# qdrant/qdrant

Hardware: NVIDIA H100
Metric: queries/sec, 10Mx768 f32 brute-force cosine top-10, single query (GB/s scanned = value * 30.72) (higher is better)
Workload: dtype f32 results (exact reference arithmetic); the scan itself runs on an int8 shadow plane and re-scores the survivors in f32

## Files before the change

qdrant_b200/csrc/qb_localk.cuh:

```cuda
#pragma once
#include "qb_common.cuh"

namespace {

constexpr int QB_LOCALK_SLOTS = 16;
constexpr int QB_LOCALK_WARPS = 8;

__device__ __forceinline__ unsigned long long warp_min_u64(unsigned long long v) {
#pragma unroll
    for (int o = 16; o > 0; o >>= 1) {
        const unsigned long long w = __shfl_xor_sync(0xFFFFFFFFu, v, o);
        v = w < v ? w : v;
    }
    return v;
}

struct LkState { unsigned long long my_key, wmin; float wthr; };
__device__ __noinline__ void lk_push(const uint32_t* deleted, const uint32_t* deleted2, uint32_t id_base, float sc, uint32_t id, unsigned long long* queue,
                                     unsigned int* count) {
    bool dead = false;
    if (deleted) dead = (deleted[id >> 5] >> (id & 31)) & 1u;
    if (deleted2) dead = dead || ((deleted2[id >> 5] >> (id & 31)) & 1u);
    if (!dead) queue[atomicAdd(count, 1u)] = qb_pack_key(sc, id + id_base);
}
__device__ __noinline__ LkState lk_drain(LkState st, const unsigned long long* queue, unsigned int* count, int lane, unsigned int n_queued) {
    for (unsigned int j = 0; j < n_queued; ++j) {
        const unsigned long long k_new = queue[j];
        if (k_new > st.wmin) {
            const unsigned int holders = __ballot_sync(0xFFFFFFFFu, st.my_key == st.wmin);
            if (lane == __ffs((int)holders) - 1) st.my_key = k_new;
            st.wmin = warp_min_u64(st.my_key);
        }
    }
    __syncwarp();
    if (lane == 0) *count = 0u;
    __syncwarp();
    st.wthr = (st.wmin != 0ull) ? qb_key_score(st.wmin) : __int_as_float(0xff800000);
    return st;
}

__device__ __forceinline__ void lk_cta_sort(unsigned long long* lists, int lane) {
    constexpr int N = QB_LOCALK_WARPS * QB_LOCALK_SLOTS;
    for (int k = 2; k <= N; k <<= 1)
        for (int j = k >> 1; j > 0; j >>= 1) {
            for (int i = lane; i < N; i += 32) {
                const int ixj = i ^ j;
                if (ixj > i) {
                    const unsigned long long a = lists[i], b = lists[ixj];
                    const bool desc = ((i & k) == 0);
                    if (desc ? (a < b) : (a > b)) { lists[i] = b; lists[ixj] = a; }
                }
            }
            __syncwarp();
        }
}

__device__ __forceinline__ void lk_last_cta_merge(const unsigned long long* all, uint32_t local_k, qb_scored_point* final_out, uint32_t* final_count,
                                                  unsigned int* done_counter, int lane) {
    __threadfence();
    __syncwarp();
    unsigned int ticket = 0;
    if (lane == 0) ticket = atomicAdd(done_counter, 1u);
    ticket = __shfl_sync(0xFFFFFFFFu, ticket, 0);
    if (ticket != gridDim.x - 1) return;
    __threadfence();
    constexpr int PER = 8;
    unsigned int pos[PER];
    unsigned long long head[PER];
#pragma unroll
    for (int i = 0; i < PER; ++i) {
        const unsigned int l = lane + 32u * i;
        pos[i] = 0;
        head[i] = (l < gridDim.x) ? __ldcg(all + (unsigned long long)l * QB_LOCALK_SLOTS) : 0ull;
    }
    unsigned int n_out = 0;
    for (unsigned int r = 0; r < local_k; ++r) {
        unsigned long long best = 0ull;
        int bi = 0;
#pragma unroll
        for (int i = 0; i < PER; ++i) if (head[i] > best) { best = head[i]; bi = i; }
        unsigned long long wbest = best;
#pragma unroll
        for (int o = 16; o > 0; o >>= 1) { const unsigned long long w = __shfl_xor_sync(0xFFFFFFFFu, wbest, o); wbest = w > wbest ? w : wbest; }
        if (wbest == 0ull) break;
        if (best == wbest) {
#pragma unroll
            for (int i = 0; i < PER; ++i)
                if (i == bi) {
                    pos[i] += 1;
                    const unsigned int l = lane + 32u * i;
                    head[i] = (pos[i] < (unsigned int)QB_LOCALK_SLOTS) ? __ldcg(all + (unsigned long long)l * QB_LOCALK_SLOTS + pos[i]) : 0ull;
                }
            qb_scored_point sp;
            sp.idx = qb_key_id(wbest); sp.score = qb_key_score(wbest);
            final_out[r] = sp;
        }
        n_out = r + 1;
    }
    if (lane == 0) { *final_count = n_out; *done_counter = 0u; }
}

}
```

qdrant_b200/csrc/qb_prefilter.cu:

```cuda
#include <algorithm>

#include "qb_internal.h"
#include "qb_localk.cuh"
#include "qb_score.cuh"

qb_status qb_dense_f32_scan_localk(const qb_storage* s, const QbScanArgs& a, uint32_t top, uint64_t* n_slots, cudaStream_t stream, uint64_t min_rows = 65536);

namespace {

constexpr int PF_CONSUMER_WARPS = 8;
constexpr int PF_MAX_PRODUCERS = 4;
constexpr int PF_PRODUCERS = 2;
constexpr int PF_THREADS = 32 * (PF_CONSUMER_WARPS + PF_MAX_PRODUCERS);
constexpr uint32_t PF_SLOT_BYTES = 12288;
constexpr uint32_t PF_CAP = 131072;
constexpr uint32_t PF_LIST_CAP = 1u << 21;

static int pf_producers() { const int o = qb_opt().prefilter_producers; return (o >= 1 && o <= PF_MAX_PRODUCERS) ? o : PF_PRODUCERS; }

struct PfParams {
    const uint8_t* rows;
    uint32_t stride;
    uint32_t row_h;
    uint32_t dim;
// ... 355 lines not shown
            if (valid) {
                *reinterpret_cast<uint16_t*>(dst + d_pad / 2 + 2 * v) = (uint16_t)hi;
                *reinterpret_cast<uint16_t*>(lo + 2 * v) = (uint16_t)lw;
            }
        }
        if (valid && t == 0) {
            float* meta = reinterpret_cast<float*>(dst + d_pad / 2 + d_pad / 8);
            meta[0] = sr;
            meta[1] = __double2float_ru(__dmul_ru(sqrt(rr5), 1.0 + 0x1p-40));
            meta[2] = __double2float_ru(__dmul_ru(sqrt(rr6), 1.0 + 0x1p-40));
            for (uint32_t b = d_pad / 2 + d_pad / 8 + 12; b < out_stride_b; ++b) dst[b] = 0;
            for (uint32_t b = d_pad / 8; b < lo_b; ++b) lo[b] = 0;
            if (bad || !(ss <= 3.0e38)) atomicOr(nonfinite, 1u);
            else atomicMax(max_norm_bits, __float_as_uint(__double2float_ru(__dmul_ru(sqrt(ss), 1.0 + 0x1p-40))));
        }
    }
}

struct Pf6Params {
    const uint8_t* rows;
    const uint8_t* lo;
    uint32_t stride;
    uint32_t d_pad;
    uint32_t dim;
    uint64_t n_rows;
    const float* q;
    uint32_t rows_per_slot, n_slots, slot_bytes;
    qb_scored_point* samp_out; uint32_t* samp_cnt; uint32_t top;
    const unsigned int* max_norm_bits;
    float* up5;
    uint64_t sample_rows;
    const uint8_t* f32_rows; uint32_t f32_stride; uint32_t id_base;
    unsigned long long* cta_keys; unsigned int* samp_ticket;
    uint32_t* list; unsigned int* list_cnt; unsigned int* list_ticket; uint32_t list_cap;
    uint32_t* cand; unsigned int* cnt; uint32_t cap;
    const uint32_t* deleted; const uint32_t* deleted2;
    int l2_keep;
};

template <int NCH>
struct Q6Query {
    uint32_t hq[NCH][4], lq[NCH][4];
    int sum_h, sum_l;
    float sq, e1, e1_5, t2a, t2b, thr_adj;
};

template <int NCH>
__device__ __forceinline__ void q6_query(const Pf6Params& p, int hl, Q6Query<NCH>& Q) {
    const uint32_t n16 = p.d_pad / 16;
    float qmax = 0.f, q1 = 0.f, q2 = 0.f;
    bool qbad = false;
#pragma unroll
    for (int c = 0; c < NCH; ++c) {
        const uint32_t v = (uint32_t)(c * 16 + hl);
#pragma unroll
        for (int k = 0; k < 16; ++k) {
            const float x = (v < n16 && v * 16 + k < p.dim) ? p.q[v * 16 + k] : 0.f;
            qbad |= !(fabsf(x) <= 3.0e38f);
            qmax = fmaxf(qmax, fabsf(x)); q1 = __fadd_ru(q1, fabsf(x)); q2 = __fmaf_rn(x, x, q2);
        }
    }
#pragma unroll
    for (int o = 8; o; o >>= 1) {
        qmax = fmaxf(qmax, __shfl_xor_sync(0xFFFFFFFFu, qmax, o)); q1 = __fadd_ru(q1, __shfl_xor_sync(0xFFFFFFFFu, q1, o)); q2 += __shfl_xor_sync(0xFFFFFFFFu, q2, o);
        qbad |= __shfl_xor_sync(0xFFFFFFFFu, (int)qbad, o) != 0;
    }
    qbad |= (qmax > 0.f && qmax < 1.0e-30f);
    const float sq = (qmax > 0.f) ? __fdiv_rn(qmax, 127.f) : 0.f;
// ... 286 lines not shown
        s += PF_CONSUMER_WARPS;
        if (s >= p.n_slots) { s -= p.n_slots; ph ^= 1u; }
    }
    if (lane < QB_LOCALK_SLOTS) lists[cw * QB_LOCALK_SLOTS + lane] = (lk.my_key == ~0ull) ? 0ull : lk.my_key;
    asm volatile("bar.sync 1, %0;" ::"n"(PF_CONSUMER_WARPS * 32) : "memory");
    if (cw == 0) lk_cta_sort(lists, lane);
    asm volatile("bar.sync 1, %0;" ::"n"(PF_CONSUMER_WARPS * 32) : "memory");
    if (cw < QB_LOCALK_SLOTS / 4) {
        const int i = cw * 4 + (lane >> 3);
        const unsigned long long k = (i < (int)p.top) ? lists[i] : 0ull;
        const uint32_t row = k ? qb_key_id(k) : 0u;
        const float sc = qbs::score_avx_group8<qbs::M_DOT>(reinterpret_cast<const float*>(p.f32_rows + (size_t)row * p.f32_stride), p.q, p.dim, lane & 7);
        if ((lane & 7) == 0) ex[i] = k ? qb_pack_key(sc, row + p.id_base) : 0ull;
    }
    asm volatile("bar.sync 1, %0;" ::"n"(PF_CONSUMER_WARPS * 32) : "memory");
    if (cw == 0) {
        if (lane < QB_LOCALK_SLOTS) {
            const unsigned long long k = ex[lane];
            int rank = 0;
#pragma unroll
            for (int j = 0; j < QB_LOCALK_SLOTS; ++j) rank += (ex[j] > k || (ex[j] == k && j < lane)) ? 1 : 0;
            p.cta_keys[(unsigned long long)blockIdx.x * QB_LOCALK_SLOTS + rank] = k;
        }
        lk_last_cta_merge(p.cta_keys, p.top, p.samp_out, p.samp_cnt, p.samp_ticket, lane);
    }
}

template <int NCH>
__global__ void __launch_bounds__(PF_THREADS, 1) dense_q5_filter_kernel(const Pf6Params p) { stage1_run<NCH, Q6Query<NCH>>(p); }

template <int NCH>
__global__ void __launch_bounds__(PF_THREADS, 1) dense_q4b_filter_kernel(const Pf6Params p) { stage1_run<NCH, Q4bQuery<NCH>>(p); }

constexpr int PF_COMPACT_THREADS = 256;
template <int NCH>
__global__ void __launch_bounds__(PF_COMPACT_THREADS) dense_q5_compact_kernel(const Pf6Params p) {
    constexpr int UNROLL = 4;
    constexpr int WARPS = PF_COMPACT_THREADS / 32;
    __shared__ float s_thr;
    __shared__ unsigned int s_warp[WARPS], s_base;
    if (threadIdx.x < 32) {
        Q6Query<NCH> Q;
        q6_query<NCH>(p, threadIdx.x & 15, Q);
        if (threadIdx.x == 0) s_thr = Q.thr_adj;
    }
    __syncthreads();
    const float thr_adj = s_thr;
    const int lane = threadIdx.x & 31, warp = threadIdx.x >> 5;
    const uint64_t n4 = (p.n_rows + 3) / 4, step = (uint64_t)gridDim.x * PF_COMPACT_THREADS * UNROLL;
    for (uint64_t b = (uint64_t)blockIdx.x * PF_COMPACT_THREADS * UNROLL; b < n4; b += step) {
        float4 u4[UNROLL];
#pragma unroll
        for (int j = 0; j < UNROLL; ++j) {
            const uint64_t i = b + (uint64_t)j * PF_COMPACT_THREADS + threadIdx.x;
            u4[j] = (i < n4) ? __ldcs(reinterpret_cast<const float4*>(p.up5) + i) : make_float4(0.f, 0.f, 0.f, 0.f);
        }
        uint32_t mask = 0;
#pragma unroll
        for (int j = 0; j < UNROLL; ++j) {
            const uint64_t i = b + (uint64_t)j * PF_COMPACT_THREADS + threadIdx.x;
            const float u[4] = {u4[j].x, u4[j].y, u4[j].z, u4[j].w};
#pragma unroll
            for (int k = 0; k < 4; ++k) {
                const uint64_t row = 4 * i + k;
                if (row < p.n_rows && !(u[k] < thr_adj)) {
                    const uint32_t id = (uint32_t)row;
                    bool dead = false;
                    if (p.deleted) dead = (p.deleted[id >> 5] >> (id & 31)) & 1u;
                    if (p.deleted2) dead = dead || ((p.deleted2[id >> 5] >> (id & 31)) & 1u);
                    mask |= dead ? 0u : 1u << (4 * j + k);
                }
            }
        }
        const int c = __popc(mask);
        int incl = c;
#pragma unroll
        for (int o = 1; o < 32; o <<= 1) { const int t = __shfl_up_sync(0xFFFFFFFFu, incl, o); if (lane >= o) incl += t; }
        if (lane == 31) s_warp[warp] = (unsigned int)incl;
        __syncthreads();
        if (threadIdx.x == 0) {
            unsigned int total = 0;
#pragma unroll
            for (int w = 0; w < WARPS; ++w) { const unsigned int t = s_warp[w]; s_warp[w] = total; total += t; }
            s_base = total ? atomicAdd(p.list_cnt, total) : 0u;
        }
        __syncthreads();
        if (mask) {
            unsigned int pos = s_base + s_warp[warp] + (unsigned int)(incl - c);
            for (uint32_t m = mask; m; m &= m - 1) {
                const int bit = __ffs((int)m) - 1;
                if (pos < p.list_cap) p.list[pos] = (uint32_t)(4 * (b + (uint64_t)(bit >> 2) * PF_COMPACT_THREADS + threadIdx.x) + (bit & 3));
                ++pos;
            }
        }
        __syncthreads();
    }
}

constexpr int PF_RESCREEN_THREADS = 256;
template <int NCH>
__global__ void __launch_bounds__(PF_RESCREEN_THREADS) dense_q6_rescreen_kernel(const Pf6Params p) {
    __shared__ uint4 s_hq[NCH * 16], s_lq[NCH * 16];
    __shared__ float s_k[5];
    __shared__ int s_corr[2];
    __shared__ unsigned int s_n;
    if (threadIdx.x == 0) {
        s_n = *reinterpret_cast<volatile unsigned int*>(p.list_cnt);
        __threadfence();
        if (atomicAdd(p.list_ticket, 1u) == gridDim.x - 1) { *p.list_cnt = 0u; *p.list_ticket = 0u; }
    }
    if (threadIdx.x < 32) {
        const int hl = threadIdx.x & 15;
        Q6Query<NCH> Q;
        q6_query<NCH>(p, hl, Q);
        if (threadIdx.x < 16) {
#pragma unroll
            for (int c = 0; c < NCH; ++c) {
                s_hq[c * 16 + hl] = make_uint4(Q.hq[c][0], Q.hq[c][1], Q.hq[c][2], Q.hq[c][3]);
                s_lq[c * 16 + hl] = make_uint4(Q.lq[c][0], Q.lq[c][1], Q.lq[c][2], Q.lq[c][3]);
            }
        }
        if (threadIdx.x == 0) {
            s_k[0] = Q.sq; s_k[1] = Q.e1; s_k[2] = Q.t2a; s_k[3] = Q.t2b; s_k[4] = Q.thr_adj;
            s_corr[0] = 31 * Q.sum_h; s_corr[1] = 31 * Q.sum_l;
        }
    }
    __syncthreads();
    const unsigned int n1 = s_n;
    if (n1 > p.list_cap) {
        if (blockIdx.x == 0 && threadIdx.x == 0) *p.cnt = p.cap + 1u;
        return;
    }
    const float sq = s_k[0], e1 = s_k[1], t2a = s_k[2], t2b = s_k[3], thr_adj = s_k[4];
    const int corr_h = s_corr[0], corr_l = s_corr[1];
    const float k254 = 1.0f / 254.0f;
    const int lane = threadIdx.x & 31, half = lane >> 4, hl = lane & 15;
    uint32_t hq[NCH][4], lq[NCH][4];
#pragma unroll
    for (int c = 0; c < NCH; ++c) {
        const uint4 h = s_hq[c * 16 + hl], l = s_lq[c * 16 + hl];
        hq[c][0] = h.x; hq[c][1] = h.y; hq[c][2] = h.z; hq[c][3] = h.w;
        lq[c][0] = l.x; lq[c][1] = l.y; lq[c][2] = l.z; lq[c][3] = l.w;
    }
    const uint32_t n16 = p.d_pad / 16, lo_b = q6_lo_stride(p.d_pad);
    const uint32_t a_off = (uint32_t)hl * 8, b_off = p.d_pad / 2 + (uint32_t)hl * 2, meta_off = p.d_pad / 2 + p.d_pad / 8;
    const uint32_t warps = gridDim.x * (blockDim.x >> 5), gw = blockIdx.x * (blockDim.x >> 5) + (threadIdx.x >> 5);
    for (uint32_t e0 = 2 * gw; e0 < n1; e0 += 2 * warps) {
        const uint32_t e = e0 + (uint32_t)half;
        const bool valid = e < n1;
        const uint32_t row = __ldcg(p.list + (valid ? e : e0));
        const uint8_t* rec = p.rows + (size_t)row * p.stride;
        const uint8_t* lo = p.lo + (size_t)row * lo_b;
        int hs = 0, ls = 0;
#pragma unroll
        for (int c = 0; c < NCH; ++c) {
            if ((uint32_t)(c * 16 + hl) < n16) {
                const uint2 x = __ldg(reinterpret_cast<const uint2*>(rec + a_off + 128 * c));
                const uint32_t y = q6_spread(__ldg(reinterpret_cast<const unsigned short*>(rec + b_off + 32 * c)));
                const uint32_t z = q6_spread(__ldg(reinterpret_cast<const unsigned short*>(lo + 2 * hl + 32 * c)));
                const uint32_t w[4] = {((x.x << 1) & 0x1E1E1E1Eu) | (y & 0x01010101u),        ((x.x >> 3) & 0x1E1E1E1Eu) | ((y >> 1) & 0x01010101u),
                                       ((x.y << 1) & 0x1E1E1E1Eu) | ((y >> 2) & 0x01010101u), ((x.y >> 3) & 0x1E1E1E1Eu) | ((y >> 3) & 0x01010101u)};
#pragma unroll
                for (int m = 0; m < 4; ++m) {
                    const uint32_t u = (w[m] << 1) | ((z >> m) & 0x01010101u);
                    hs = __dp4a((int)u, (int)hq[c][m], hs); ls = __dp4a((int)u, (int)lq[c][m], ls);
                }
            }
        }
        int v = ((hl & 8) ? ls : hs) + __shfl_xor_sync(0xFFFFFFFFu, (hl & 8) ? hs : ls, 8);
        v += __shfl_xor_sync(0xFFFFFFFFu, v, 4);
        v += __shfl_xor_sync(0xFFFFFFFFu, v, 2);
        v += __shfl_xor_sync(0xFFFFFFFFu, v, 1);
        const int lsum = __shfl_xor_sync(0xFFFFFFFFu, v, 8);
        if (hl == 0 && valid) {
            const float* meta = reinterpret_cast<const float*>(rec + meta_off);
            const float H = (float)(v - corr_h), L = (float)(lsum - corr_l);
            const float sr = __ldg(meta), rho6 = __ldg(meta + 2);
            const float app = __fmul_rn(sr, __fmul_rn(sq, __fmaf_rn(L, k254, H)));
            const float up = __fadd_ru(app, fminf(__fmul_ru(sr, e1), __fmaf_ru(rho6, t2a, t2b)));
            if (!(up < thr_adj)) {
                const unsigned int pos = atomicAdd(p.cnt, 1u);
                if (pos < p.cap) p.cand[pos] = row;
            }
        }
    }
}

template <typename P>
qb_status launch_ring(void (*kernel)(P), P& p, int sm_count, cudaStream_t stream, size_t extra_smem = 0, uint32_t row_step = 2) {
    const uint32_t kMaxSmem = 227 * 1024;
    const uint32_t target = qb_opt().prefilter_slot_bytes ? qb_opt().prefilter_slot_bytes : PF_SLOT_BYTES;
    uint32_t rps = target / p.stride / row_step * row_step;
    if (rps < row_step) rps = row_step;
    p.rows_per_slot = rps;
    p.slot_bytes = rps * p.stride;
    uint32_t n_slots = (kMaxSmem - 2048 - (uint32_t)extra_smem) / p.slot_bytes;
    if (n_slots > 64) n_slots = 64;
    n_slots = (n_slots / PF_CONSUMER_WARPS) * PF_CONSUMER_WARPS;
    QB_CHECK(n_slots >= (uint32_t)PF_CONSUMER_WARPS, QB_ERR_INVALID, "prefilter: rows too wide for the ring");
    p.n_slots = n_slots;
    const size_t smem = (size_t)n_slots * p.slot_bytes + (size_t)n_slots * 16 + extra_smem;
    QB_CUDA(cudaFuncSetAttribute(kernel, cudaFuncAttributeMaxDynamicSharedMemorySize, (int)kMaxSmem));
    const uint64_t n_tiles = ceil_div_u64(p.n_rows, p.rows_per_slot);
    const unsigned grid = (unsigned)std::min<uint64_t>(n_tiles, (uint64_t)sm_count);
    kernel<<<grid, 32 * (PF_CONSUMER_WARPS + pf_producers()), smem, stream>>>(p);
    QB_LAUNCHED();
    QB_CUDA(cudaGetLastError());
    return QB_OK;
}

template <bool GLOBAL>
__device__ unsigned long long block_next_key(const unsigned long long* k, uint32_t n, unsigned long long prev, unsigned long long* s_best) {
    const int warp = threadIdx.x >> 5, lane = threadIdx.x & 31;
    unsigned long long best = 0ull;
    for (uint32_t i = threadIdx.x; i < n; i += blockDim.x) {
        const unsigned long long x = GLOBAL ? __ldcg(k + i) : k[i];
        if (x < prev && x > best) best = x;
    }
#pragma unroll
    for (int o = 16; o; o >>= 1) { const unsigned long long w = __shfl_xor_sync(0xFFFFFFFFu, best, o); best = w > best ? w : best; }
// ... 116 lines not shown
    }
    s->q4b_row_b = row_b;
    const uint64_t blocks = std::min<uint64_t>(ceil_div_u64(std::max<uint64_t>(s->count, 1), 32), (uint64_t)s->sm_count * 16);
    f32_to_q4b_rows_kernel<<<(unsigned)blocks, 256, 0, stream>>>(reinterpret_cast<const float*>(s->d_rows), s->row_stride / 4, s->dim, d_pad, s->count, s->d_q4b, row_b);
    QB_LAUNCHED();
    QB_CUDA(cudaGetLastError());
    QB_CUDA(cudaStreamSynchronize(stream));
    s->q4b_ready = true;
    return QB_OK;
}

static bool pf_stage1_q4b() { return qb_opt().prefilter_stage1 != 5; }

static int pf_plane() { const int o = qb_opt().prefilter_plane; return (o == 1 || o == 2) ? o : 0; }

bool qb_f32_prefilter_usable(qb_storage* s, uint64_t n_rows, uint32_t top, cudaStream_t stream) {
    if (s->kind != QB_KIND_DENSE || s->dtype != QB_DT_F32) return false;
    if (s->distance != QB_DIST_DOT && s->distance != QB_DIST_COSINE) return false;
    if (qb_opt().disable_prefilter || n_rows != s->count || n_rows < (1ull << 19) || top > 16 || s->dim < 32 || round_up_u64(s->dim, 8) > 1024) return false;
    if (pf_plane() == 0) {
        if (q6_shadow_ensure(s, stream) == QB_OK) {
            if (s->q6_usable && pf_stage1_q4b() && q4b_shadow_ensure(s, stream) != QB_OK) cudaGetLastError();
            return s->q6_usable;
        }
        cudaGetLastError();
    } else if (pf_plane() == 2) {
        if (q8_shadow_ensure(s, stream) == QB_OK) return s->q8_usable;
        cudaGetLastError();
    }
    if (qb_f32_shadow_ensure(s, stream) != QB_OK) { cudaGetLastError(); return false; }
    return s->bf16_usable;
}

size_t qb_f32_prefilter_scratch_bytes() { return 256 + (size_t)PF_CAP * 12 + (size_t)PF_LIST_CAP * 4; }

qb_status qb_f32_prefilter_search(qb_storage* s, const QbScanArgs& a, uint32_t top, void* d_scratch, float* d_up5, unsigned int* d_n_fallbacks, qb_scored_point* d_out,
                                  uint32_t* d_out_cnt, cudaEvent_t prof0, cudaEvent_t prof1, cudaStream_t stream) {
    uint8_t* sc = reinterpret_cast<uint8_t*>(d_scratch);
    unsigned int* d_cnt = reinterpret_cast<unsigned int*>(sc);
    unsigned int* d_fallback = reinterpret_cast<unsigned int*>(sc + 16);
    uint32_t* d_samp_cnt = reinterpret_cast<uint32_t*>(sc + 48);
    qb_scored_point* d_samp = reinterpret_cast<qb_scored_point*>(sc + 64);
    unsigned int* d_ticket = reinterpret_cast<unsigned int*>(sc + 32);
    unsigned int* d_list_cnt = reinterpret_cast<unsigned int*>(sc + 192);
    unsigned int* d_list_ticket = reinterpret_cast<unsigned int*>(sc + 208);
    unsigned int* d_samp_ticket = reinterpret_cast<unsigned int*>(sc + 224);
    unsigned long long* d_keys = reinterpret_cast<unsigned long long*>(sc + 256);
    uint32_t* d_cand = reinterpret_cast<uint32_t*>(d_keys + PF_CAP);
    uint32_t* d_list = d_cand + PF_CAP;
    const uint64_t n = s->count;
    const uint32_t cap = (uint32_t)std::min<uint64_t>(PF_CAP, n / 32);
    const float* d_q = reinterpret_cast<const float*>(a.d_q_enc);
    const int plane = pf_plane();
    uint64_t n_slots = 0;
    if (plane == 0 && s->q6_ready && s->q6_usable) {
        uint64_t sample = n / 8;
        if (qb_opt().sample_rows) sample = std::min<uint64_t>(n, std::max<uint64_t>(16384, qb_opt().sample_rows & ~(uint64_t)3));
        Pf6Params p6{};
        p6.rows = s->d_q6; p6.lo = s->d_q6_lo; p6.stride = s->q6_row_b; p6.d_pad = (uint32_t)round_up_u64(s->dim, 32); p6.dim = s->dim; p6.n_rows = n;
        p6.q = d_q; p6.samp_out = d_samp; p6.samp_cnt = d_samp_cnt; p6.top = top; p6.max_norm_bits = s->d_q6_meta;
        p6.up5 = d_up5; p6.sample_rows = sample;
        p6.f32_rows = reinterpret_cast<const uint8_t*>(s->d_rows); p6.f32_stride = s->row_stride; p6.id_base = a.emit.id_base;
        p6.cta_keys = d_keys; p6.samp_ticket = d_samp_ticket;
        p6.list = d_list; p6.list_cnt = d_list_cnt; p6.list_ticket = d_list_ticket; p6.list_cap = (uint32_t)std::min<uint64_t>(PF_LIST_CAP, n);
        p6.cand = d_cand; p6.cnt = d_cnt; p6.cap = cap; p6.deleted = a.emit.deleted; p6.deleted2 = a.emit.deleted2;
        p6.l2_keep = ((uint64_t)n * p6.stride <= (64ull << 20)) ? 1 : 0;
        const unsigned cp_grid = (unsigned)s->sm_count * 8, rs_grid = (unsigned)s->sm_count * 4;
        QB_CHECK((uint64_t)s->sm_count * QB_LOCALK_SLOTS <= PF_CAP, QB_ERR_INVALID, "prefilter: %d CTAs exceed the key buffer", s->sm_count);
        if (prof0) cudaEventRecord(prof0, stream);
        if (pf_stage1_q4b() && s->q4b_ready) {
            Pf6Params p4 = p6;
            p4.rows = s->d_q4b; p4.stride = s->q4b_row_b;
            switch ((p4.d_pad + 255) / 256) {
                case 1: QB_TRY(launch_ring(dense_q4b_filter_kernel<1>, p4, s->sm_count, stream, PF_SAMPLE_SMEM, 4)); break;
                case 2: QB_TRY(launch_ring(dense_q4b_filter_kernel<2>, p4, s->sm_count, stream, PF_SAMPLE_SMEM, 4)); break;
                case 3: QB_TRY(launch_ring(dense_q4b_filter_kernel<3>, p4, s->sm_count, stream, PF_SAMPLE_SMEM, 4)); break;
                default: QB_TRY(launch_ring(dense_q4b_filter_kernel<4>, p4, s->sm_count, stream, PF_SAMPLE_SMEM, 4)); break;
            }
        } else {
            switch ((p6.d_pad + 255) / 256) {
                case 1: QB_TRY(launch_ring(dense_q5_filter_kernel<1>, p6, s->sm_count, stream, PF_SAMPLE_SMEM, 4)); break;
                case 2: QB_TRY(launch_ring(dense_q5_filter_kernel<2>, p6, s->sm_count, stream, PF_SAMPLE_SMEM, 4)); break;
                case 3: QB_TRY(launch_ring(dense_q5_filter_kernel<3>, p6, s->sm_count, stream, PF_SAMPLE_SMEM, 4)); break;
                default: QB_TRY(launch_ring(dense_q5_filter_kernel<4>, p6, s->sm_count, stream, PF_SAMPLE_SMEM, 4)); break;
            }
        }
        if (prof1) cudaEventRecord(prof1, stream);
        switch ((p6.d_pad + 255) / 256) {
            case 1: dense_q5_compact_kernel<1><<<cp_grid, PF_COMPACT_THREADS, 0, stream>>>(p6); dense_q6_rescreen_kernel<1><<<rs_grid, PF_RESCREEN_THREADS, 0, stream>>>(p6); break;
            case 2: dense_q5_compact_kernel<2><<<cp_grid, PF_COMPACT_THREADS, 0, stream>>>(p6); dense_q6_rescreen_kernel<2><<<rs_grid, PF_RESCREEN_THREADS, 0, stream>>>(p6); break;
            case 3: dense_q5_compact_kernel<3><<<cp_grid, PF_COMPACT_THREADS, 0, stream>>>(p6); dense_q6_rescreen_kernel<3><<<rs_grid, PF_RESCREEN_THREADS, 0, stream>>>(p6); break;
            default: dense_q5_compact_kernel<4><<<cp_grid, PF_COMPACT_THREADS, 0, stream>>>(p6); dense_q6_rescreen_kernel<4><<<rs_grid, PF_RESCREEN_THREADS, 0, stream>>>(p6); break;
        }
        QB_LAUNCHED();
        QB_LAUNCHED();
        QB_CUDA(cudaGetLastError());
    } else {
    uint64_t sample = std::min<uint64_t>(131072, std::max<uint64_t>(16384, (n / 64) & ~(uint64_t)3));
    if (qb_opt().sample_rows) sample = std::min<uint64_t>(n, std::max<uint64_t>(16384, qb_opt().sample_rows & ~(uint64_t)3));
    QbScanArgs as = a;
    as.row_begin = 0; as.row_end = sample;
    as.emit.final_out = d_samp; as.emit.final_count = d_samp_cnt; as.emit.run_if = nullptr;
    QB_TRY(qb_dense_f32_scan_localk(s, as, top, &n_slots, stream, 4096));
    QB_CHECK(n_slots != 0 && n_slots <= 4096, QB_ERR_CUDA, "prefilter: the sample scan did not launch (%llu slots)", (unsigned long long)n_slots);
    if (plane == 2 && s->q8_ready && s->q8_usable) {
        Pf8Params p8{};
        p8.rows = reinterpret_cast<const uint8_t*>(s->d_q8); p8.stride = s->q8_row_b; p8.dim = s->dim; p8.n_rows = n;
        p8.q = d_q; p8.samp_out = d_samp; p8.samp_cnt = d_samp_cnt; p8.top = top; p8.max_norm_bits = s->d_q8_meta;
        p8.cand = d_cand; p8.cnt = d_cnt; p8.cap = cap; p8.deleted = a.emit.deleted; p8.deleted2 = a.emit.deleted2;
        p8.l2_keep = ((uint64_t)n * p8.stride <= (64ull << 20)) ? 1 : 0;
        if (prof0) cudaEventRecord(prof0, stream);
        switch ((p8.stride - 16 + 255) / 256) {
            case 1: QB_TRY(launch_ring(dense_q8_filter_kernel<1>, p8, s->sm_count, stream)); break;
            case 2: QB_TRY(launch_ring(dense_q8_filter_kernel<2>, p8, s->sm_count, stream)); break;
            case 3: QB_TRY(launch_ring(dense_q8_filter_kernel<3>, p8, s->sm_count, stream)); break;
            default: QB_TRY(launch_ring(dense_q8_filter_kernel<4>, p8, s->sm_count, stream)); break;
        }
        if (prof1) cudaEventRecord(prof1, stream);
    } else {
    PfParams p{};
    p.rows = reinterpret_cast<const uint8_t*>(s->d_bf16); p.row_h = s->bf16_row_h; p.stride = s->bf16_row_h * 2; p.dim = s->dim; p.n_rows = n;
    p.q = reinterpret_cast<const float*>(a.d_q_enc);
    p.samp_out = d_samp; p.samp_cnt = d_samp_cnt; p.top = top; p.max_norm_bits = s->d_bf16_meta;
    p.cand = d_cand; p.cnt = d_cnt; p.cap = cap; p.deleted = a.emit.deleted; p.deleted2 = a.emit.deleted2;
    p.l2_keep = ((uint64_t)n * p.stride <= (64ull << 20)) ? 1 : 0;
    if (prof0) cudaEventRecord(prof0, stream);
    const uint32_t nch = (p.row_h + 255) / 256;
    switch (nch) {
        case 1: QB_TRY(launch_ring(dense_bf16_filter_kernel<1>, p, s->sm_count, stream)); break;
        case 2: QB_TRY(launch_ring(dense_bf16_filter_kernel<2>, p, s->sm_count, stream)); break;
        case 3: QB_TRY(launch_ring(dense_bf16_filter_kernel<3>, p, s->sm_count, stream)); break;
        default: QB_TRY(launch_ring(dense_bf16_filter_kernel<4>, p, s->sm_count, stream)); break;
    }
    if (prof1) cudaEventRecord(prof1, stream);
    }
    }
    const unsigned fin_grid = (unsigned)std::max<uint32_t>((uint32_t)s->sm_count, ceil_div_u64(PF_CAP, 4096));
    const size_t fin_smem = (size_t)ceil_div_u64(cap, fin_grid) * sizeof(unsigned long long);
    QB_CHECK((uint64_t)fin_grid * top <= PF_CAP, QB_ERR_INVALID, "prefilter: %u finish CTAs x top %u exceed the key buffer", fin_grid, top);
    f32_prefilter_finish_kernel<<<fin_grid, PF_FINISH_THREADS, fin_smem, stream>>>(reinterpret_cast<const uint8_t*>(s->d_rows), s->row_stride, s->dim, d_q, d_cand, d_cnt, cap,
                                                                                   top, a.emit.id_base, d_keys, d_ticket, d_out, d_out_cnt, d_fallback, d_n_fallbacks);
    QB_LAUNCHED();
    QB_CUDA(cudaGetLastError());
    QbScanArgs af = a;
    af.row_begin = 0; af.row_end = n;
    af.emit.final_out = d_out; af.emit.final_count = d_out_cnt; af.emit.run_if = d_fallback;
    QB_TRY(qb_dense_f32_scan_localk(s, af, top, &n_slots, stream));
    QB_CHECK(n_slots != 0 && n_slots <= 4096, QB_ERR_CUDA, "prefilter: the fallback scan did not launch (%llu slots)", (unsigned long long)n_slots);
    return QB_OK;
}
```

Before: 566.0.

## Fuse compact, rescreen and f32 rescore into one select kernel with local top-k

Replaces the compact, q6 rescreen and separate f32 finish kernels on the q6 path with a single select kernel. Each CTA reads its bound slice, queues passing rows in shared memory, rescreens them with the q6 dot product, and rescores survivors in f32 into a per-warp top-k. A last-CTA merge then writes the final top-k. The global candidate list buffer and the finish kernel launch go away, which saves launches and global round trips at the cost of heavier per-CTA work and extra shared memory. It also adds L2 prefetches and an early-stop path that hands off to the fallback scan.

```diff
diff --git a/qdrant_b200/csrc/qb_localk.cuh b/qdrant_b200/csrc/qb_localk.cuh
--- a/qdrant_b200/csrc/qb_localk.cuh
+++ b/qdrant_b200/csrc/qb_localk.cuh
@@ -55,23 +55,16 @@
         }
 }
 
-__device__ __forceinline__ void lk_last_cta_merge(const unsigned long long* all, uint32_t local_k, qb_scored_point* final_out, uint32_t* final_count,
-                                                  unsigned int* done_counter, int lane) {
-    __threadfence();
-    __syncwarp();
-    unsigned int ticket = 0;
-    if (lane == 0) ticket = atomicAdd(done_counter, 1u);
-    ticket = __shfl_sync(0xFFFFFFFFu, ticket, 0);
-    if (ticket != gridDim.x - 1) return;
-    __threadfence();
-    constexpr int PER = 8;
+template <int PER, class Emit>
+__device__ __forceinline__ unsigned int lk_merge_heads(const unsigned long long* all, unsigned int first, unsigned int step, unsigned int n_lists, uint32_t local_k,
+                                                       int lane, Emit emit) {
     unsigned int pos[PER];
     unsigned long long head[PER];
 #pragma unroll
     for (int i = 0; i < PER; ++i) {
-        const unsigned int l = lane + 32u * i;
+        const unsigned int l = first + step * (lane + 32u * i);
         pos[i] = 0;
-        head[i] = (l < gridDim.x) ? __ldcg(all + (unsigned long long)l * QB_LOCALK_SLOTS) : 0ull;
+        head[i] = (l < n_lists) ? __ldcg(all + (unsigned long long)l * QB_LOCALK_SLOTS) : 0ull;
     }
     unsigned int n_out = 0;
     for (unsigned int r = 0; r < local_k; ++r) {
@@ -88,15 +81,30 @@
             for (int i = 0; i < PER; ++i)
                 if (i == bi) {
                     pos[i] += 1;
-                    const unsigned int l = lane + 32u * i;
+                    const unsigned int l = first + step * (lane + 32u * i);
                     head[i] = (pos[i] < (unsigned int)QB_LOCALK_SLOTS) ? __ldcg(all + (unsigned long long)l * QB_LOCALK_SLOTS + pos[i]) : 0ull;
                 }
-            qb_scored_point sp;
-            sp.idx = qb_key_id(wbest); sp.score = qb_key_score(wbest);
-            final_out[r] = sp;
+            emit(r, wbest);
         }
         n_out = r + 1;
     }
+    return n_out;
+}
+
+__device__ __forceinline__ void lk_last_cta_merge(const unsigned long long* all, uint32_t local_k, qb_scored_point* final_out, uint32_t* final_count,
+                                                  unsigned int* done_counter, int lane) {
+    __threadfence();
+    __syncwarp();
+    unsigned int ticket = 0;
+    if (lane == 0) ticket = atomicAdd(done_counter, 1u);
+    ticket = __shfl_sync(0xFFFFFFFFu, ticket, 0);
+    if (ticket != gridDim.x - 1) return;
+    __threadfence();
+    const unsigned int n_out = lk_merge_heads<8>(all, 0u, 1u, gridDim.x, local_k, lane, [&](unsigned int r, unsigned long long k) {
+        qb_scored_point sp;
+        sp.idx = qb_key_id(k); sp.score = qb_key_score(k);
+        final_out[r] = sp;
+    });
     if (lane == 0) { *final_count = n_out; *done_counter = 0u; }
 }
 
diff --git a/qdrant_b200/csrc/qb_prefilter.cu b/qdrant_b200/csrc/qb_prefilter.cu
--- a/qdrant_b200/csrc/qb_prefilter.cu
+++ b/qdrant_b200/csrc/qb_prefilter.cu
@@ -411,8 +411,9 @@
     uint64_t sample_rows;
     const uint8_t* f32_rows; uint32_t f32_stride; uint32_t id_base;
     unsigned long long* cta_keys; unsigned int* samp_ticket;
-    uint32_t* list; unsigned int* list_cnt; unsigned int* list_ticket; uint32_t list_cap;
-    uint32_t* cand; unsigned int* cnt; uint32_t cap;
+    unsigned int* list_cnt; unsigned int* list_ticket; uint32_t list_cap;
+    unsigned int* cnt; uint32_t cap;
+    qb_scored_point* out; uint32_t* out_cnt; unsigned int* fallback; unsigned int* n_fallbacks;
     const uint32_t* deleted; const uint32_t* deleted2;
     int l2_keep;
 };
@@ -765,38 +766,102 @@
 template <int NCH>
 __global__ void __launch_bounds__(PF_THREADS, 1) dense_q4b_filter_kernel(const Pf6Params p) { stage1_run<NCH, Q4bQuery<NCH>>(p); }
 
-constexpr int PF_COMPACT_THREADS = 256;
+constexpr int PF_SELECT_THREADS = 32 * QB_LOCALK_WARPS;
+__host__ __device__ constexpr int pf_select_ctas_per_sm(int nch) { return nch == 3 ? 4 : nch == 4 ? 2 : 3; }
+constexpr int PF_SELECT_UNROLL = 8;
+constexpr uint32_t PF_SELECT_WARP_ROWS = 32 * 4 * PF_SELECT_UNROLL;
+constexpr uint32_t PF_SELECT_SURV = 64;
+constexpr int PF_SELECT_MERGE_PER = 4;
+
+__device__ __forceinline__ void pf_prefetch_bounds(const float* up5, uint32_t w0, uint32_t end, int lane) {
+    const uint32_t i = w0 + (uint32_t)lane * 8;
+    if (lane < 16 && i < end) asm volatile("prefetch.global.L2 [%0];" ::"l"(reinterpret_cast<const float4*>(up5) + i));
+}
+__device__ __forceinline__ void pf_prefetch_rows(const uint8_t* base, uint32_t stride, uint32_t bytes, const uint32_t* ids, uint32_t n, int lane) {
+    const uint32_t per = (bytes + 127) / 128 + 1;
+    for (uint32_t t = (uint32_t)lane; t < n * per; t += 32) {
+        const uint32_t e = t / per, k = t - e * per;
+        asm volatile("prefetch.global.L2 [%0];" ::"l"(base + (size_t)ids[e] * stride + min(k * 128, bytes - 1)));
+    }
+}
 template <int NCH>
-__global__ void __launch_bounds__(PF_COMPACT_THREADS) dense_q5_compact_kernel(const Pf6Params p) {
-    constexpr int UNROLL = 4;
-    constexpr int WARPS = PF_COMPACT_THREADS / 32;
-    __shared__ float s_thr;
-    __shared__ unsigned int s_warp[WARPS], s_base;
-    if (threadIdx.x < 32) {
+__global__ void __launch_bounds__(PF_SELECT_THREADS, pf_select_ctas_per_sm(NCH)) dense_q6_select_kernel(const Pf6Params p) {
+    __shared__ uint4 s_hq[NCH * 16], s_lq[NCH * 16];
+    __shared__ float s_k[5];
+    __shared__ int s_corr[2];
+    __shared__ uint32_t s_queue[QB_LOCALK_WARPS * PF_SELECT_WARP_ROWS];
+    __shared__ uint32_t s_surv[QB_LOCALK_WARPS][PF_SELECT_SURV];
+    __shared__ unsigned long long s_lists[QB_LOCALK_WARPS * QB_LOCALK_SLOTS];
+    __shared__ unsigned long long s_lkq[QB_LOCALK_WARPS][4];
+    __shared__ unsigned int s_lkc[QB_LOCALK_WARPS], s_qn[2], s_total, s_ticket;
+    __shared__ int s_stop, s_bad;
+    const int warp = threadIdx.x >> 5, lane = threadIdx.x & 31, half = lane >> 4, hl = lane & 15;
+    if (warp == 0) {
         Q6Query<NCH> Q;
-        q6_query<NCH>(p, threadIdx.x & 15, Q);
-        if (threadIdx.x == 0) s_thr = Q.thr_adj;
-    }
+        q6_query<NCH>(p, hl, Q);
+        if (lane < 16) {
+#pragma unroll
+            for (int c = 0; c < NCH; ++c) {
+                s_hq[c * 16 + hl] = make_uint4(Q.hq[c][0], Q.hq[c][1], Q.hq[c][2], Q.hq[c][3]);
+                s_lq[c * 16 + hl] = make_uint4(Q.lq[c][0], Q.lq[c][1], Q.lq[c][2], Q.lq[c][3]);
+            }
+        }
+        if (lane == 0) {
+            s_k[0] = Q.sq; s_k[1] = Q.e1; s_k[2] = Q.t2a; s_k[3] = Q.t2b; s_k[4] = Q.thr_adj;
+            s_corr[0] = 31 * Q.sum_h; s_corr[1] = 31 * Q.sum_l;
+        }
+    }
+    if (threadIdx.x < QB_LOCALK_WARPS) s_lkc[threadIdx.x] = 0u;
+    if (threadIdx.x < 2) s_qn[threadIdx.x] = 0u;
+    constexpr uint32_t STEP = QB_LOCALK_WARPS * (PF_SELECT_WARP_ROWS / 4);
+    const uint32_t n4 = (uint32_t)((p.n_rows + 3) / 4), per = (n4 + gridDim.x - 1) / gridDim.x;
+    const uint32_t begin = min(n4, blockIdx.x * per), end = min(n4, begin + per);
+    pf_prefetch_bounds(p.up5, begin + (uint32_t)warp * (PF_SELECT_WARP_ROWS / 4), end, lane);
     __syncthreads();
-    const float thr_adj = s_thr;
-    const int lane = threadIdx.x & 31, warp = threadIdx.x >> 5;
-    const uint64_t n4 = (p.n_rows + 3) / 4, step = (uint64_t)gridDim.x * PF_COMPACT_THREADS * UNROLL;
-    for (uint64_t b = (uint64_t)blockIdx.x * PF_COMPACT_THREADS * UNROLL; b < n4; b += step) {
-        float4 u4[UNROLL];
-#pragma unroll
-        for (int j = 0; j < UNROLL; ++j) {
-            const uint64_t i = b + (uint64_t)j * PF_COMPACT_THREADS + threadIdx.x;
-            u4[j] = (i < n4) ? __ldcs(reinterpret_cast<const float4*>(p.up5) + i) : make_float4(0.f, 0.f, 0.f, 0.f);
-        }
+    const float thr_adj = s_k[4];
+    uint32_t* surv = s_surv[warp];
+    uint32_t n_surv = 0;
+    LkState lk{(lane < (int)p.top) ? 0ull : ~0ull, 0ull, __int_as_float(0xff800000)};
+    auto flush = [&]() {
+        pf_prefetch_rows(p.f32_rows, p.f32_stride, p.dim * 4, surv, n_surv, lane);
+        unsigned int old = 0;
+        if (lane == 0) old = atomicAdd(p.cnt, n_surv);
+        old = __shfl_sync(0xFFFFFFFFu, old, 0);
+        if (old + n_surv <= p.cap) {
+            for (uint32_t s0 = 0; s0 < n_surv; s0 += 4) {
+                const uint32_t i = s0 + (uint32_t)(lane >> 3);
+                const uint32_t row = surv[i < n_surv ? i : s0];
+                const float sc = qbs::score_avx_group8<qbs::M_DOT>(reinterpret_cast<const float*>(p.f32_rows + (size_t)row * p.f32_stride), p.q, p.dim, lane & 7);
+                if (i < n_surv && (lane & 7) == 0 && !(sc < lk.wthr)) lk_push(nullptr, nullptr, p.id_base, sc, row, s_lkq[warp], &s_lkc[warp]);
+                __syncwarp();
+                const unsigned int n_queued = *reinterpret_cast<volatile unsigned int*>(&s_lkc[warp]);
+                if (n_queued) lk = lk_drain(lk, s_lkq[warp], &s_lkc[warp], lane, n_queued);
+            }
+        }
+        __syncwarp();
+        n_surv = 0;
+    };
+    bool stopped = false;
+    for (uint32_t b = begin, it = 0; b < end; b += STEP, ++it) {
+        unsigned int seen_l = 0, seen_c = 0;
+        if (threadIdx.x == 0) { seen_l = *reinterpret_cast<volatile unsigned int*>(p.list_cnt); seen_c = *reinterpret_cast<volatile unsigned int*>(p.cnt); }
+        const uint32_t w0 = b + (uint32_t)warp * (PF_SELECT_WARP_ROWS / 4);
+        float4 u4[PF_SELECT_UNROLL];
+#pragma unroll
+        for (int j = 0; j < PF_SELECT_UNROLL; ++j) {
+            const uint32_t i = w0 + (uint32_t)j * 32 + lane;
+            u4[j] = (i < end) ? __ldcs(reinterpret_cast<const float4*>(p.up5) + i) : make_float4(0.f, 0.f, 0.f, 0.f);
+        }
+        pf_prefetch_bounds(p.up5, w0 + STEP, end, lane);
         uint32_t mask = 0;
 #pragma unroll
-        for (int j = 0; j < UNROLL; ++j) {
-            const uint64_t i = b + (uint64_t)j * PF_COMPACT_THREADS + threadIdx.x;
+        for (int j = 0; j < PF_SELECT_UNROLL; ++j) {
+            const uint32_t i = w0 + (uint32_t)j * 32 + lane;
             const float u[4] = {u4[j].x, u4[j].y, u4[j].z, u4[j].w};
 #pragma unroll
             for (int k = 0; k < 4; ++k) {
-                const uint64_t row = 4 * i + k;
-                if (row < p.n_rows && !(u[k] < thr_adj)) {
+                const uint64_t row = 4 * (uint64_t)i + k;
+                if (i < end && row < p.n_rows && !(u[k] < thr_adj)) {
                     const uint32_t id = (uint32_t)row;
                     bool dead = false;
                     if (p.deleted) dead = (p.deleted[id >> 5] >> (id & 31)) & 1u;
@@ -805,120 +870,131 @@
                 }
             }
         }
-        const int c = __popc(mask);
-        int incl = c;
+        const int nc = __popc(mask);
+        int incl = nc;
 #pragma unroll
         for (int o = 1; o < 32; o <<= 1) { const int t = __shfl_up_sync(0xFFFFFFFFu, incl, o); if (lane >= o) incl += t; }
-        if (lane == 31) s_warp[warp] = (unsigned int)incl;
+        unsigned int base = 0;
+        if (lane == 31 && incl) base = atomicAdd(&s_qn[it & 1], (unsigned int)incl);
+        base = __shfl_sync(0xFFFFFFFFu, base, 31);
+        {
+            uint32_t pos = base + (uint32_t)(incl - nc);
+            for (uint32_t m = mask; m; m &= m - 1) {
+                const int bit = __ffs((int)m) - 1;
+                s_queue[pos++] = 4 * (w0 + (uint32_t)(bit >> 2) * 32 + lane) + (uint32_t)(bit & 3);
+            }
+        }
         __syncthreads();
         if (threadIdx.x == 0) {
-            unsigned int total = 0;
-#pragma unroll
-            for (int w = 0; w < WARPS; ++w) { const unsigned int t = s_warp[w]; s_warp[w] = total; total += t; }
-            s_base = total ? atomicAdd(p.list_cnt, total) : 0u;
+            const unsigned int total = s_qn[it & 1];
+            if (total) atomicAdd(p.list_cnt, total);
+            s_total = total;
+            s_qn[(it & 1) ^ 1] = 0u;
+            s_stop = (seen_l + total > p.list_cap || seen_c > p.cap) ? 1 : 0;
         }
         __syncthreads();
-        if (mask) {
-            unsigned int pos = s_base + s_warp[warp] + (unsigned int)(incl - c);
-            for (uint32_t m = mask; m; m &= m - 1) {
-                const int bit = __ffs((int)m) - 1;
-                if (pos < p.list_cap) p.list[pos] = (uint32_t)(4 * (b + (uint64_t)(bit >> 2) * PF_COMPACT_THREADS + threadIdx.x) + (bit & 3));
-                ++pos;
-            }
-        }
-        __syncthreads();
-    }
-}
-
-constexpr int PF_RESCREEN_THREADS = 256;
-template <int NCH>
-__global__ void __launch_bounds__(PF_RESCREEN_THREADS) dense_q6_rescreen_kernel(const Pf6Params p) {
-    __shared__ uint4 s_hq[NCH * 16], s_lq[NCH * 16];
-    __shared__ float s_k[5];
-    __shared__ int s_corr[2];
-    __shared__ unsigned int s_n;
+        if (s_stop) { stopped = true; break; }
+        const uint32_t nq = s_total;
+        for (uint32_t e0 = (uint32_t)warp * 4; e0 < nq; e0 += 4 * QB_LOCALK_WARPS) {
+            const uint32_t ea = e0 + (uint32_t)half, eb = ea + 2;
+            const bool va = ea < nq, vb = eb < nq;
+            const uint32_t ra = s_queue[va ? ea : e0], rb = s_queue[vb ? eb : e0];
+            const uint32_t n16 = p.d_pad / 16, lo_b = q6_lo_stride(p.d_pad);
+            const uint32_t a_off = (uint32_t)hl * 8, b_off = p.d_pad / 2 + (uint32_t)hl * 2, meta_off = p.d_pad / 2 + p.d_pad / 8;
+            const uint8_t* reca = p.rows + (size_t)ra * p.stride;
+            const uint8_t* recb = p.rows + (size_t)rb * p.stride;
+            const uint8_t* loa = p.lo + (size_t)ra * lo_b;
+            const uint8_t* lob = p.lo + (size_t)rb * lo_b;
+            uint2 xa[NCH], xb[NCH];
+            uint32_t ya[NCH], yb[NCH], za[NCH], zb[NCH];
+#pragma unroll
+            for (int c = 0; c < NCH; ++c) {
+                const bool in = (uint32_t)(c * 16 + hl) < n16;
+                xa[c] = in ? __ldg(reinterpret_cast<const uint2*>(reca + a_off + 128 * c)) : make_uint2(0u, 0u);
+                xb[c] = in ? __ldg(reinterpret_cast<const uint2*>(recb + a_off + 128 * c)) : make_uint2(0u, 0u);
+                ya[c] = in ? __ldg(reinterpret_cast<const unsigned short*>(reca + b_off + 32 * c)) : 0u;
+                yb[c] = in ? __ldg(reinterpret_cast<const unsigned short*>(recb + b_off + 32 * c)) : 0u;
+                za[c] = in ? __ldg(reinterpret_cast<const unsigned short*>(loa + 2 * hl + 32 * c)) : 0u;
+                zb[c] = in ? __ldg(reinterpret_cast<const unsigned short*>(lob + 2 * hl + 32 * c)) : 0u;
+            }
+            const float* meta = reinterpret_cast<const float*>(((hl & 4) ? recb : reca) + meta_off);
+            const float sr = __ldg(meta), rho6 = __ldg(meta + 2);
+            int ha = 0, la = 0, hb = 0, lb = 0;
+#pragma unroll
+            for (int c = 0; c < NCH; ++c) {
+                const uint4 h4 = s_hq[c * 16 + hl], l4 = s_lq[c * 16 + hl];
+                const uint32_t hq[4] = {h4.x, h4.y, h4.z, h4.w}, lq[4] = {l4.x, l4.y, l4.z, l4.w};
+                const uint32_t ysa = q6_spread(ya[c]), ysb = q6_spread(yb[c]), zsa = q6_spread(za[c]), zsb = q6_spread(zb[c]);
+                const uint32_t wa[4] = {((xa[c].x << 1) & 0x1E1E1E1Eu) | (ysa & 0x01010101u),        ((xa[c].x >> 3) & 0x1E1E1E1Eu) | ((ysa >> 1) & 0x01010101u),
+                                        ((xa[c].y << 1) & 0x1E1E1E1Eu) | ((ysa >> 2) & 0x01010101u), ((xa[c].y >> 3) & 0x1E1E1E1Eu) | ((ysa >> 3) & 0x01010101u)};
+                const uint32_t wb[4] = {((xb[c].x << 1) & 0x1E1E1E1Eu) | (ysb & 0x01010101u),        ((xb[c].x >> 3) & 0x1E1E1E1Eu) | ((ysb >> 1) & 0x01010101u),
+                                        ((xb[c].y << 1) & 0x1E1E1E1Eu) | ((ysb >> 2) & 0x01010101u), ((xb[c].y >> 3) & 0x1E1E1E1Eu) | ((ysb >> 3) & 0x01010101u)};
+#pragma unroll
+                for (int m = 0; m < 4; ++m) {
+                    const uint32_t ua = (wa[m] << 1) | ((zsa >> m) & 0x01010101u), ub = (wb[m] << 1) | ((zsb >> m) & 0x01010101u);
+                    ha = __dp4a((int)ua, (int)hq[m], ha); la = __dp4a((int)ua, (int)lq[m], la);
+                    hb = __dp4a((int)ub, (int)hq[m], hb); lb = __dp4a((int)ub, (int)lq[m], lb);
+                }
+            }
+            const int x0 = ((hl & 8) ? la : ha) + __shfl_xor_sync(0xFFFFFFFFu, (hl & 8) ? ha : la, 8);
+            const int x1 = ((hl & 8) ? lb : hb) + __shfl_xor_sync(0xFFFFFFFFu, (hl & 8) ? hb : lb, 8);
+            int v = ((hl & 4) ? x1 : x0) + __shfl_xor_sync(0xFFFFFFFFu, (hl & 4) ? x0 : x1, 4);
+            v += __shfl_xor_sync(0xFFFFFFFFu, v, 2);
+            v += __shfl_xor_sync(0xFFFFFFFFu, v, 1);
+            const int lsum = __shfl_xor_sync(0xFFFFFFFFu, v, 8);
+            bool pass = false;
+            if ((hl == 0 && va) || (hl == 4 && vb)) {
+                const float sq = s_k[0], e1 = s_k[1], t2a = s_k[2], t2b = s_k[3], k254 = 1.0f / 254.0f;
+                const float H = (float)(v - s_corr[0]), L = (float)(lsum - s_corr[1]);
+                const float app = __fmul_rn(sr, __fmul_rn(sq, __fmaf_rn(L, k254, H)));
+                const float up = __fadd_ru(app, fminf(__fmul_ru(sr, e1), __fmaf_ru(rho6, t2a, t2b)));
+                pass = !(up < thr_adj);
+            }
+            const uint32_t pm = __ballot_sync(0xFFFFFFFFu, pass);
+            if (pass) surv[n_surv + __popc(pm & ((1u << lane) - 1u))] = hl ? rb : ra;
+            n_surv += (uint32_t)__popc(pm);
+            if (n_surv > PF_SELECT_SURV - 4) { __syncwarp(); flush(); }
+        }
+        __syncwarp();
+    }
+    if (!stopped && n_surv) { __syncwarp(); flush(); }
+    if (lane < QB_LOCALK_SLOTS) s_lists[warp * QB_LOCALK_SLOTS + lane] = (lk.my_key == ~0ull) ? 0ull : lk.my_key;
+    __syncthreads();
+    if (warp == 0) {
+        lk_cta_sort(s_lists, lane);
+        if (lane < QB_LOCALK_SLOTS) p.cta_keys[(size_t)blockIdx.x * QB_LOCALK_SLOTS + lane] = s_lists[lane];
+        __threadfence();
+        __syncwarp();
+        if (lane == 0) s_ticket = atomicAdd(p.list_ticket, 1u);
+    }
+    __syncthreads();
+    if (s_ticket != gridDim.x - 1) return;
+    __threadfence();
     if (threadIdx.x == 0) {
-        s_n = *reinterpret_cast<volatile unsigned int*>(p.list_cnt);
-        __threadfence();
-        if (atomicAdd(p.list_ticket, 1u) == gridDim.x - 1) { *p.list_cnt = 0u; *p.list_ticket = 0u; }
-    }
-    if (threadIdx.x < 32) {
-        const int hl = threadIdx.x & 15;
-        Q6Query<NCH> Q;
-        q6_query<NCH>(p, hl, Q);
-        if (threadIdx.x < 16) {
-#pragma unroll
-            for (int c = 0; c < NCH; ++c) {
-                s_hq[c * 16 + hl] = make_uint4(Q.hq[c][0], Q.hq[c][1], Q.hq[c][2], Q.hq[c][3]);
-                s_lq[c * 16 + hl] = make_uint4(Q.lq[c][0], Q.lq[c][1], Q.lq[c][2], Q.lq[c][3]);
-            }
-        }
-        if (threadIdx.x == 0) {
-            s_k[0] = Q.sq; s_k[1] = Q.e1; s_k[2] = Q.t2a; s_k[3] = Q.t2b; s_k[4] = Q.thr_adj;
-            s_corr[0] = 31 * Q.sum_h; s_corr[1] = 31 * Q.sum_l;
-        }
-    }
+        const unsigned int n1 = __ldcg(p.list_cnt), cnt = __ldcg(p.cnt);
+        const bool bad = n1 > p.list_cap || cnt > p.cap || cnt < p.top;
+        *p.list_cnt = 0u; *p.cnt = 0u; *p.list_ticket = 0u;
+        *p.fallback = bad ? 1u : 0u;
+        if (bad) atomicAdd(p.n_fallbacks, 1u);
+        s_bad = bad ? 1 : 0;
+    }
+    if (lane < QB_LOCALK_SLOTS) s_lists[warp * QB_LOCALK_SLOTS + lane] = 0ull;
     __syncthreads();
-    const unsigned int n1 = s_n;
-    if (n1 > p.list_cap) {
-        if (blockIdx.x == 0 && threadIdx.x == 0) *p.cnt = p.cap + 1u;
-        return;
-    }
-    const float sq = s_k[0], e1 = s_k[1], t2a = s_k[2], t2b = s_k[3], thr_adj = s_k[4];
-    const int corr_h = s_corr[0], corr_l = s_corr[1];
-    const float k254 = 1.0f / 254.0f;
-    const int lane = threadIdx.x & 31, half = lane >> 4, hl = lane & 15;
-    uint32_t hq[NCH][4], lq[NCH][4];
-#pragma unroll
-    for (int c = 0; c < NCH; ++c) {
-        const uint4 h = s_hq[c * 16 + hl], l = s_lq[c * 16 + hl];
-        hq[c][0] = h.x; hq[c][1] = h.y; hq[c][2] = h.z; hq[c][3] = h.w;
-        lq[c][0] = l.x; lq[c][1] = l.y; lq[c][2] = l.z; lq[c][3] = l.w;
-    }
-    const uint32_t n16 = p.d_pad / 16, lo_b = q6_lo_stride(p.d_pad);
-    const uint32_t a_off = (uint32_t)hl * 8, b_off = p.d_pad / 2 + (uint32_t)hl * 2, meta_off = p.d_pad / 2 + p.d_pad / 8;
-    const uint32_t warps = gridDim.x * (blockDim.x >> 5), gw = blockIdx.x * (blockDim.x >> 5) + (threadIdx.x >> 5);
-    for (uint32_t e0 = 2 * gw; e0 < n1; e0 += 2 * warps) {
-        const uint32_t e = e0 + (uint32_t)half;
-        const bool valid = e < n1;
-        const uint32_t row = __ldcg(p.list + (valid ? e : e0));
-        const uint8_t* rec = p.rows + (size_t)row * p.stride;
-        const uint8_t* lo = p.lo + (size_t)row * lo_b;
-        int hs = 0, ls = 0;
-#pragma unroll
-        for (int c = 0; c < NCH; ++c) {
-            if ((uint32_t)(c * 16 + hl) < n16) {
-                const uint2 x = __ldg(reinterpret_cast<const uint2*>(rec + a_off + 128 * c));
-                const uint32_t y = q6_spread(__ldg(reinterpret_cast<const unsigned short*>(rec + b_off + 32 * c)));
-                const uint32_t z = q6_spread(__ldg(reinterpret_cast<const unsigned short*>(lo + 2 * hl + 32 * c)));
-                const uint32_t w[4] = {((x.x << 1) & 0x1E1E1E1Eu) | (y & 0x01010101u),        ((x.x >> 3) & 0x1E1E1E1Eu) | ((y >> 1) & 0x01010101u),
-                                       ((x.y << 1) & 0x1E1E1E1Eu) | ((y >> 2) & 0x01010101u), ((x.y >> 3) & 0x1E1E1E1Eu) | ((y >> 3) & 0x01010101u)};
-#pragma unroll
-                for (int m = 0; m < 4; ++m) {
-                    const uint32_t u = (w[m] << 1) | ((z >> m) & 0x01010101u);
-                    hs = __dp4a((int)u, (int)hq[c][m], hs); ls = __dp4a((int)u, (int)lq[c][m], ls);
-                }
-            }
-        }
-        int v = ((hl & 8) ? ls : hs) + __shfl_xor_sync(0xFFFFFFFFu, (hl & 8) ? hs : ls, 8);
-        v += __shfl_xor_sync(0xFFFFFFFFu, v, 4);
-        v += __shfl_xor_sync(0xFFFFFFFFu, v, 2);
-        v += __shfl_xor_sync(0xFFFFFFFFu, v, 1);
-        const int lsum = __shfl_xor_sync(0xFFFFFFFFu, v, 8);
-        if (hl == 0 && valid) {
-            const float* meta = reinterpret_cast<const float*>(rec + meta_off);
-            const float H = (float)(v - corr_h), L = (float)(lsum - corr_l);
-            const float sr = __ldg(meta), rho6 = __ldg(meta + 2);
-            const float app = __fmul_rn(sr, __fmul_rn(sq, __fmaf_rn(L, k254, H)));
-            const float up = __fadd_ru(app, fminf(__fmul_ru(sr, e1), __fmaf_ru(rho6, t2a, t2b)));
-            if (!(up < thr_adj)) {
-                const unsigned int pos = atomicAdd(p.cnt, 1u);
-                if (pos < p.cap) p.cand[pos] = row;
-            }
-        }
-    }
-}
-
+    if (s_bad) return;
+    lk_merge_heads<PF_SELECT_MERGE_PER>(p.cta_keys, (unsigned int)warp, (unsigned int)QB_LOCALK_WARPS, gridDim.x, p.top, lane,
+                                        [&](unsigned int r, unsigned long long k) { s_lists[warp * QB_LOCALK_SLOTS + r] = k; });
+    __syncthreads();
+    if (warp == 0) {
+        lk_cta_sort(s_lists, lane);
+        if (lane < (int)p.top) {
+            const unsigned long long k = s_lists[lane];
+            qb_scored_point sp;
+            sp.idx = qb_key_id(k); sp.score = qb_key_score(k);
+            p.out[lane] = sp;
+        }
+        if (lane == 0) *p.out_cnt = p.top;
+    }
+}
 template <typename P>
 qb_status launch_ring(void (*kernel)(P), P& p, int sm_count, cudaStream_t stream, size_t extra_smem = 0, uint32_t row_step = 2) {
     const uint32_t kMaxSmem = 227 * 1024;
@@ -1101,7 +1177,7 @@
     return s->bf16_usable;
 }
 
-size_t qb_f32_prefilter_scratch_bytes() { return 256 + (size_t)PF_CAP * 12 + (size_t)PF_LIST_CAP * 4; }
+size_t qb_f32_prefilter_scratch_bytes() { return 256 + (size_t)PF_CAP * 12; }
 
 qb_status qb_f32_prefilter_search(qb_storage* s, const QbScanArgs& a, uint32_t top, void* d_scratch, float* d_up5, unsigned int* d_n_fallbacks, qb_scored_point* d_out,
                                   uint32_t* d_out_cnt, cudaEvent_t prof0, cudaEvent_t prof1, cudaStream_t stream) {
@@ -1116,7 +1192,6 @@
     unsigned int* d_samp_ticket = reinterpret_cast<unsigned int*>(sc + 224);
     unsigned long long* d_keys = reinterpret_cast<unsigned long long*>(sc + 256);
     uint32_t* d_cand = reinterpret_cast<uint32_t*>(d_keys + PF_CAP);
-    uint32_t* d_list = d_cand + PF_CAP;
     const uint64_t n = s->count;
     const uint32_t cap = (uint32_t)std::min<uint64_t>(PF_CAP, n / 32);
     const float* d_q = reinterpret_cast<const float*>(a.d_q_enc);
@@ -1131,11 +1206,13 @@
         p6.up5 = d_up5; p6.sample_rows = sample;
         p6.f32_rows = reinterpret_cast<const uint8_t*>(s->d_rows); p6.f32_stride = s->row_stride; p6.id_base = a.emit.id_base;
         p6.cta_keys = d_keys; p6.samp_ticket = d_samp_ticket;
-        p6.list = d_list; p6.list_cnt = d_list_cnt; p6.list_ticket = d_list_ticket; p6.list_cap = (uint32_t)std::min<uint64_t>(PF_LIST_CAP, n);
-        p6.cand = d_cand; p6.cnt = d_cnt; p6.cap = cap; p6.deleted = a.emit.deleted; p6.deleted2 = a.emit.deleted2;
+        p6.list_cnt = d_list_cnt; p6.list_ticket = d_list_ticket; p6.list_cap = (uint32_t)std::min<uint64_t>(PF_LIST_CAP, n);
+        p6.cnt = d_cnt; p6.cap = cap; p6.deleted = a.emit.deleted; p6.deleted2 = a.emit.deleted2;
+        p6.out = d_out; p6.out_cnt = d_out_cnt; p6.fallback = d_fallback; p6.n_fallbacks = d_n_fallbacks;
         p6.l2_keep = ((uint64_t)n * p6.stride <= (64ull << 20)) ? 1 : 0;
-        const unsigned cp_grid = (unsigned)s->sm_count * 8, rs_grid = (unsigned)s->sm_count * 4;
-        QB_CHECK((uint64_t)s->sm_count * QB_LOCALK_SLOTS <= PF_CAP, QB_ERR_INVALID, "prefilter: %d CTAs exceed the key buffer", s->sm_count);
+        const unsigned sel_grid = (unsigned)s->sm_count * pf_select_ctas_per_sm((p6.d_pad + 255) / 256);
+        QB_CHECK((uint64_t)sel_grid * QB_LOCALK_SLOTS <= PF_CAP && sel_grid <= 32u * PF_SELECT_MERGE_PER * QB_LOCALK_WARPS, QB_ERR_INVALID,
+                 "prefilter: %d SMs exceed the key buffer", s->sm_count);
         if (prof0) cudaEventRecord(prof0, stream);
         if (pf_stage1_q4b() && s->q4b_ready) {
             Pf6Params p4 = p6;
@@ -1156,12 +1233,11 @@
         }
         if (prof1) cudaEventRecord(prof1, stream);
         switch ((p6.d_pad + 255) / 256) {
-            case 1: dense_q5_compact_kernel<1><<<cp_grid, PF_COMPACT_THREADS, 0, stream>>>(p6); dense_q6_rescreen_kernel<1><<<rs_grid, PF_RESCREEN_THREADS, 0, stream>>>(p6); break;
-            case 2: dense_q5_compact_kernel<2><<<cp_grid, PF_COMPACT_THREADS, 0, stream>>>(p6); dense_q6_rescreen_kernel<2><<<rs_grid, PF_RESCREEN_THREADS, 0, stream>>>(p6); break;
-            case 3: dense_q5_compact_kernel<3><<<cp_grid, PF_COMPACT_THREADS, 0, stream>>>(p6); dense_q6_rescreen_kernel<3><<<rs_grid, PF_RESCREEN_THREADS, 0, stream>>>(p6); break;
-            default: dense_q5_compact_kernel<4><<<cp_grid, PF_COMPACT_THREADS, 0, stream>>>(p6); dense_q6_rescreen_kernel<4><<<rs_grid, PF_RESCREEN_THREADS, 0, stream>>>(p6); break;
-        }
-        QB_LAUNCHED();
+            case 1: dense_q6_select_kernel<1><<<sel_grid, PF_SELECT_THREADS, 0, stream>>>(p6); break;
+            case 2: dense_q6_select_kernel<2><<<sel_grid, PF_SELECT_THREADS, 0, stream>>>(p6); break;
+            case 3: dense_q6_select_kernel<3><<<sel_grid, PF_SELECT_THREADS, 0, stream>>>(p6); break;
+            default: dense_q6_select_kernel<4><<<sel_grid, PF_SELECT_THREADS, 0, stream>>>(p6); break;
+        }
         QB_LAUNCHED();
         QB_CUDA(cudaGetLastError());
     } else {
@@ -1203,7 +1279,6 @@
     }
     if (prof1) cudaEventRecord(prof1, stream);
     }
-    }
     const unsigned fin_grid = (unsigned)std::max<uint32_t>((uint32_t)s->sm_count, ceil_div_u64(PF_CAP, 4096));
     const size_t fin_smem = (size_t)ceil_div_u64(cap, fin_grid) * sizeof(unsigned long long);
     QB_CHECK((uint64_t)fin_grid * top <= PF_CAP, QB_ERR_INVALID, "prefilter: %u finish CTAs x top %u exceed the key buffer", fin_grid, top);
@@ -1211,6 +1286,7 @@
                                                                                    top, a.emit.id_base, d_keys, d_ticket, d_out, d_out_cnt, d_fallback, d_n_fallbacks);
     QB_LAUNCHED();
     QB_CUDA(cudaGetLastError());
+    }
     QbScanArgs af = a;
     af.row_begin = 0; af.row_end = n;
     af.emit.final_out = d_out; af.emit.final_count = d_out_cnt; af.emit.run_if = d_fallback;
```

Result: faster. 579.3 (median of 6 runs) (+2.3%).
